# Borda/pyImSegm

Hardware: AMD Instinct MI355X
Metric: Mpixels/s end-to-end SLIC+fts+GC, 2048x2048 RGB; % HBM roofline (higher is better)
Workload: dtype f64; 1 GPU; single 2048x2048 RGB uint8 per GPU, SLIC(sp_size=46, K=2025, 10 sweeps) + colour mean/std/energy + 3-class alpha-expansion GC (gc_regul=2.0, edge=model), pre-fitted GMM, host numpy in -> segm int32 in host numpy (BASELINE configs[1]); bench_config=2, images_per_launch_chain=1, images_in_flight_per_gpu=4, hardware_queues=4, input_memory=pageable numpy, input_ring=default (one rank: measured in round 4), parallelism=images sharded over 1 GPU(s), 4 in flight per GPU (one HIP stream each)

## Files before the change

### pyimsegm_amd/build.py

```python
import os
import subprocess
import sys

HERE = os.path.dirname(os.path.abspath(__file__))
CSRC = os.path.join(HERE, 'csrc')
LIB = os.path.join(HERE, 'libimsegm_hip.so')
SOURCES = ['api.hip', 'api_image2d.hip', 'api_texture.hip', 'api_volume.hip', 'api_fused.hip', 'api_natives.hip', 'batch.hip', 'slic_pre.hip', 'slic.hip', 'connectivity.hip', 'stats.hip', 'graph.hip', 'graphcut.hip', 'texture.hip', 'volume.hip', 'terms.hip', 'natives.hip', 'median.hip', 'output.hip']
HEADERS = ['common.h', 'slic.h', 'session.h', os.path.join('..', '..', 'include', 'imsegm_hip.h')]
FLAGS = ['--offload-arch=gfx950', '-O3', '-std=c++17', '-fPIC', '-ffp-contract=off', '-fvisibility=hidden',
         '-Wall', '-Wno-unused-function', '-Wno-pass-failed']


def _stale(target, deps):
    if not os.path.exists(target):
        return True
    t = os.path.getmtime(target)
    return any(os.path.getmtime(d) > t for d in deps)


def build(force=False, verbose=True):
    hipcc = os.environ.get('HIPCC', '/opt/rocm/bin/hipcc')
    objdir = os.path.join(HERE, 'build')
    os.makedirs(objdir, exist_ok=True)
    headers = [os.path.join(CSRC, h) for h in HEADERS]
    objs = []
    procs = []
    for src in SOURCES:
        spath = os.path.join(CSRC, src)
        obj = os.path.join(objdir, src.replace('.hip', '.o'))
        objs.append(obj)
        if force or _stale(obj, [spath] + headers):
            cmd = [hipcc] + FLAGS + ['-c', spath, '-o', obj]
            if verbose:
                print(' '.join(cmd), flush=True)
            procs.append((src, subprocess.Popen(cmd)))
    for src, p in procs:
        if p.wait() != 0:
            raise RuntimeError('hipcc failed on %s' % src)
    if force or procs or _stale(LIB, objs):
        cmd = [hipcc, '--offload-arch=gfx950', '-shared', '-fPIC', '-o', LIB] + objs
        if verbose:
            print(' '.join(cmd), flush=True)
        subprocess.check_call(cmd)
    return LIB


if __name__ == '__main__':
    build(force='--force' in sys.argv)
```

### pyimsegm_amd/csrc/api.hip

```cpp
#include "../../include/imsegm_hip.h"
#include "slic.h"

#include <atomic>
#include <cstdio>
#include <cstdlib>
#include <cstring>
#include <vector>

namespace imsegm {

static thread_local std::string g_error;

void set_error(const std::string &msg) { g_error = msg; }

bool hip_ok(hipError_t e, const char *what, const char *file, int line)
{
    if (e == hipSuccess) return true;
    char buf[512];
    snprintf(buf, sizeof(buf), "HIP error %d (%s) in `%s` at %s:%d", (int)e, hipGetErrorString(e), what, file, line);
    g_error = buf;
    return false;
}

static Knobs read_knobs()
{
    auto flag = [](const char *n) { return getenv(n) != nullptr; };
    auto num = [](const char *n, int dflt) { const char *e = getenv(n); return e ? atoi(e) : dflt; };
    Knobs k;
    k.slic_graph = flag("IMSEGM_SLIC_GRAPH");
    k.pre_3pass = flag("IMSEGM_PRE_3PASS");
    k.separate_finalize = flag("IMSEGM_SEPARATE_FINALIZE");
    k.fuse_finalize = flag("IMSEGM_FUSE_FINALIZE");
    k.conn_general = flag("IMSEGM_CONN_GENERAL");
    k.gc_no_topo_regs = flag("IMSEGM_GC_NO_TOPO_REGS");
    k.sep_wide_tile = flag("IMSEGM_SEP_WIDE_TILE");
    k.cc_merge_full = flag("IMSEGM_CC_MERGE_FULL");
    k.label_general = flag("IMSEGM_LABEL_GENERAL");
    k.terms_one_workgroup = flag("IMSEGM_TERMS_ONE_WORKGROUP");
    k.adjacency_table = flag("IMSEGM_ADJACENCY_TABLE");
    k.brick_cap = num("IMSEGM_BRICK_CAP", 0);
    k.gc_lds_level = num("IMSEGM_GC_LDS_LEVEL", 4);
    k.gc_threads = num("IMSEGM_GC_THREADS", 0);
    k.gc_grid_min_sites = num("IMSEGM_GC_GRID_MIN_SITES", 0);
    k.gc_grid_blocks = num("IMSEGM_GC_GRID_BLOCKS", 0);
    k.gc_one_workgroup = flag("IMSEGM_GC_ONE_WORKGROUP");
    k.gc_grid_test_absent = flag("IMSEGM_GC_GRID_TEST_ABSENT");
    k.fused_bitmap_mb = num("IMSEGM_FUSED_BITMAP_MB", 0);
    const char *d = getenv("IMSEGM_PHASE_DUMP");
    k.phase_dump = d ? d : "";
    return k;
}
static std::atomic<const Knobs *> g_knobs{ nullptr };
const Knobs &knobs()
{
    const Knobs *k = g_knobs.load(std::memory_order_acquire);
    if (!k) {
        const Knobs *fresh = new Knobs(read_knobs());
        if (g_knobs.compare_exchange_strong(k, fresh, std::memory_order_acq_rel)) k = fresh;
        else delete fresh;
    }
    return *k;
}
void reload_knobs() { g_knobs.store(new Knobs(read_knobs()), std::memory_order_release); }

}

#include "session.h"

std::atomic<bool> g_runtime_started{ false };

extern "C" {

int imsegm_host_alloc(size_t bytes, void **ptr_out)
{
    g_runtime_started.store(true);
    if (!ptr_out) {
        set_error("null argument");
        return -1;
    }
    HIP_TRY(hipHostMalloc(ptr_out, bytes ? bytes : 1, hipHostMallocDefault));
    return 0;
}

void imsegm_host_free(void *ptr)
{
    if (ptr) (void)hipHostFree(ptr);
}

int imsegm_device_alloc(int device, size_t bytes, void **ptr_out)
{
    g_runtime_started.store(true);
    if (!ptr_out) {
        set_error("null argument");
        return -1;
    }
    HIP_TRY(hipSetDevice(device));
    HIP_TRY(hipMalloc(ptr_out, bytes ? bytes : 1));
    return 0;
}

void imsegm_device_free(void *ptr)
{
    if (ptr) (void)hipFree(ptr);
}

int imsegm_set_device(int device)
{
    g_runtime_started.store(true);
    HIP_TRY(hipSetDevice(device));
    return 0;
}

int imsegm_ctx_stream(imsegm_ctx *ctx, void **stream_out)
{
    if (bind(ctx)) return -1;
    *stream_out = ctx->stream;
    return 0;
}

int imsegm_ctx_copy(imsegm_ctx *ctx, void *dst, const void *src, size_t bytes, int synchronize)
{
    if (bind(ctx)) return -1;
    HIP_TRY(hipMemcpyAsync(dst, src, bytes, hipMemcpyDefault, ctx->stream));
    if (synchronize) HIP_TRY(hipStreamSynchronize(ctx->stream));
    return 0;
}

const char *imsegm_last_error(void) { return g_error.c_str(); }
int imsegm_version(void) { return 100; }

// ... 59 lines not shown
    ctx->device = device;
    HIP_TRY(hipStreamCreateWithFlags(&ctx->stream, hipStreamNonBlocking));
    *ctx_out = ctx;
    return 0;
}

void imsegm_ctx_destroy(imsegm_ctx *ctx)
{
    if (!ctx) return;
    (void)hipSetDevice(ctx->device);
    ctx->collect();
    for (auto e : ctx->pool) (void)hipEventDestroy(e);
    ctx->gc_buf.release();
    ctx->aux_buf.release();
    if (ctx->pinned_ev) (void)hipEventDestroy(ctx->pinned_ev);
    if (ctx->pinned) (void)hipHostFree(ctx->pinned);
    if (ctx->stream) (void)hipStreamDestroy(ctx->stream);
    delete ctx;
}

int imsegm_ctx_synchronize(imsegm_ctx *ctx)
{
    if (bind(ctx)) return -1;
    HIP_TRY(hipStreamSynchronize(ctx->stream));
    return 0;
}

int imsegm_ctx_profile_enable(imsegm_ctx *ctx, int enable)
{
    if (bind(ctx)) return -1;
    ctx->collect();
    ctx->profile = enable != 0;
    return 0;
}

int imsegm_ctx_profile_reset(imsegm_ctx *ctx)
{
    if (bind(ctx)) return -1;
    ctx->collect();
    for (int i = 0; i < PG_COUNT; ++i) {
        ctx->acc_ms[i] = 0;
        ctx->acc_n[i] = 0;
    }
    return 0;
}

int imsegm_ctx_profile_get(imsegm_ctx *ctx, int group, double *total_ms_out, int *count_out)
{
    if (bind(ctx)) return -1;
    if (group < 0 || group >= PG_COUNT) {
        set_error("bad profile group");
        return -1;
    }
    ctx->collect();
    *total_ms_out = ctx->acc_ms[group];
    *count_out = ctx->acc_n[group];
    return 0;
}

int imsegm_image2d_create(imsegm_ctx *ctx, int height, int width, imsegm_image2d **img_out)
{
    if (bind(ctx)) return -1;
    if (height <= 0 || width <= 0 || (long)height * width > 0x3fffffffL) {
        set_error("bad image size");
        return -1;
    }
    imsegm_image2d *im = new imsegm_image2d();
    im->ctx = ctx;
    im->H = height;
    im->W = width;
    im->n = (size_t)height * width;
    *img_out = im;
    return 0;
}

void imsegm_image2d_destroy(imsegm_image2d *im)
{
    if (!im) return;
    (void)hipSetDevice(im->ctx->device);
    (void)hipStreamSynchronize(im->ctx->stream);
    DevBuf *all[] = { &im->img, &im->labA, &im->labB, &im->nearest, &im->labels, &im->conn_i32, &im->conn_u8, &im->small,
                      &im->cent, &im->tiles, &im->feat, &im->graph, &im->gather_lut, &im->gather_out_i, &im->gather_out_f,
                      &im->tex_planes, &im->tex_resp, &im->tex_small, &im->vol_cent, &im->annot, &im->hist, &im->featK, &im->seg,
                      &im->gseg, &im->narrow };
    for (auto b : all) b->release();
    if (im->slic_fail_host) (void)hipHostFree(im->slic_fail_host);
    if (im->slic_exec) (void)hipGraphExecDestroy(im->slic_exec);
    delete im;
}

int imsegm_image2d_upload(imsegm_image2d *im, const void *host_pixels, int dtype)
{
    if (!im || bind(im->ctx)) return -1;
    if (wrong_kind(im, false)) return -1;
    im->tex_ready = false;
    size_t es = dtype == IMSEGM_U8 ? 1 : dtype == IMSEGM_F32 ? 4 : dtype == IMSEGM_F64 ? 8 : 0;
    if (!es) {
        set_error("unsupported dtype");
        return -1;
    }
    size_t bytes = im->n * 3 * es;
    if (im->img.ensure(bytes + 16)) return -1;
    HIP_TRY(hipMemcpyAsync(im->img.p, host_pixels, bytes, hipMemcpyHostToDevice, im->ctx->stream));
    if (!is_pinned(host_pixels)) HIP_TRY(hipStreamSynchronize(im->ctx->stream));
    im->dtype = dtype;
    im->feat_mask = 0;
    im->place_F = 0;
    return 0;
}

long imsegm_debug_conn_general_runs(void) { return conn_general_runs(); }

void imsegm_debug_reload_env(void) { reload_knobs(); }

long imsegm_debug_gc_grid_fallbacks(void) { return gc_grid_fallbacks(); }

int imsegm_debug_slic_sweep_runs(long *persistent_runs_out, long *fallback_runs_out)
{
    slic_sweep_counters(persistent_runs_out, fallback_runs_out);
    return 0;
}

int imsegm_image2d_all_finite(imsegm_image2d *im, int *all_finite_out)
{
    if (!im || !all_finite_out || bind(im->ctx)) return -1;
    if (im->dtype < 0 || !im->img.p) {
        set_error("all_finite needs an uploaded image or volume");
        return -1;
    }
    *all_finite_out = 1;
    if (im->dtype == IMSEGM_U8) return 0;
    hipStream_t st = im->ctx->stream;
    if (ensure_small(im)) return -1;
    unsigned int *count = reinterpret_cast<unsigned int *>(im->small.as<unsigned char>() + 256);
    const size_t values = im->is_volume ? im->n : im->n * 3;
    if (launch_count_nonfinite(im->img.p, im->dtype, values, count, st)) return -1;
    unsigned int bad = 0;
    HIP_TRY(hipMemcpyAsync(&bad, count, sizeof(bad), hipMemcpyDeviceToHost, st));
    HIP_TRY(hipStreamSynchronize(st));
    *all_finite_out = bad == 0;
    return 0;
}

int imsegm_image2d_device_ptr(imsegm_image2d *im, int which, void **ptr_out)
{
    if (!im || !ptr_out) {
        set_error("null argument");
        return -1;
    }
    DevBuf *b = which == 0 ? &im->labels : which == 1 ? &im->gather_out_i : which == 2 ? &im->gather_out_f : nullptr;
    if (!b || !b->p) {
        set_error("device_ptr: buffer not available");
        return -1;
    }
    *ptr_out = b->p;
    return 0;
}


}
```

### pyimsegm_amd/csrc/api_fused.hip

```cpp
#include "session.h"

extern "C" {

int imsegm_cut_general_graph(imsegm_ctx *ctx, const int32_t *edges, int n_edges, const double *edge_weights,
                             const double *unary_cost, int n_sites, int n_labels, const double *pairwise_cost,
                             int n_iter, int32_t *labels_out, int64_t *energy_out)
{
    if (bind(ctx)) return -1;
    const int K = n_sites, C = n_labels, E = n_edges;
    if (K < 1 || C < 1 || E < 0) {
        set_error("cut_general_graph: bad sizes");
        return -1;
    }
    for (int j = 0; j < E; ++j) {
        int a = edges[2 * j], b = edges[2 * j + 1];
        if (a < 0 || b >= K || a >= b) {
            set_error("cut_general_graph: edges must satisfy 0 <= edges[:,0] < edges[:,1] < n_sites");
            return -1;
        }
    }
    for (int a = 0; a < C; ++a)
        for (int b = 0; b < C; ++b)
            if (pairwise_cost[a * C + b] != pairwise_cost[b * C + a]) {
                set_error("Cost matrix not square or not symmetric");
// ... 409 lines not shown
        return -1;
    }
    memset(host, 0, up_bytes);
    reinterpret_cast<int32_t *>(host + o_misc)[0] = K;
    memcpy(host + o_pw, pairwise, (size_t)C * C * 8);
    int32_t *si = reinterpret_cast<int32_t *>(host + o_sm);
    int smax = 0;
    double pmax = -DBL_MAX;
    for (int i = 0; i < C * C; ++i) {
        si[i] = (int32_t)(pairwise[i] * 100);
        smax = std::max(smax, std::abs(si[i]));
        pmax = std::max(pmax, pairwise[i]);
    }
    const int metric = smooth_is_metric(si, C);
    if (classes_lut) memcpy(host + o_cl, classes_lut, (size_t)C * 4);
    if (gmm) {
        if (gmm->scaler_mean) memcpy(host + o_sc, gmm->scaler_mean, (size_t)F * 8);
        if (gmm->scaler_scale) memcpy(host + o_sc + (size_t)F * 8, gmm->scaler_scale, (size_t)F * 8);
        memcpy(host + o_pc, gmm->prec_chol, (size_t)C * FF * 8);
        memcpy(host + o_mp, gmm->mu_proj, (size_t)C * F * 8);
        memcpy(host + o_ld, gmm->log_det, (size_t)C * 8);
        memcpy(host + o_lw, gmm->log_weights, (size_t)C * 8);
    } else {
        memcpy(host + o_pr, proba, (size_t)K * C * 8);
    }
    HIP_TRY(hipMemcpyAsync(dev + d_par, host, up_bytes, hipMemcpyHostToDevice, st));
    ctx->mark_stage_in_flight();
    int32_t *misc = reinterpret_cast<int32_t *>(dev + d_misc);
    int32_t *K_dev = misc, *E_dev = misc + 1, *status = misc + 2;
    long long *energy = reinterpret_cast<long long *>(dev + d_misc + 16);
    double *scalars = reinterpret_cast<double *>(dev + d_misc + 64);
    if (prepared) E_dev = nullptr;
    else if (graph_enqueue(im, g, K_dev, E_dev)) return -1;
    unsigned char *gb = im->gseg.as<unsigned char>();
    int32_t *ghead = reinterpret_cast<int32_t *>(gb + g.o_head);
    if (!E_dev) E_dev = ghead + 1;
    int32_t *edges = reinterpret_cast<int32_t *>(gb + g.o_edges);
    double *centres = reinterpret_cast<double *>(gb + g.o_cent);
    int32_t *arc_start = reinterpret_cast<int32_t *>(gb + g.o_as), *arc_to = reinterpret_cast<int32_t *>(gb + g.o_at);
    int32_t *arc_rev = reinterpret_cast<int32_t *>(gb + g.o_ar), *edge_arc = reinterpret_cast<int32_t *>(gb + g.o_ea);
    TermsArgs a;
    memset(&a, 0, sizeof(a));
    a.Kp = K_dev; a.K_cap = K; a.Ep = E_dev; a.edge_capacity = Ecap; a.F = F; a.C = C;
    a.features = need_features ? im->featK.as<double>() : nullptr;
    a.gmm = gmm ? 1 : 0;
    if (gmm) {
        a.scaler_mean = gmm->scaler_mean ? reinterpret_cast<double *>(dev + d_par + o_sc) : nullptr;
        a.scaler_scale = gmm->scaler_scale ? reinterpret_cast<double *>(dev + d_par + o_sc) + F : nullptr;
        a.prec_chol = reinterpret_cast<double *>(dev + d_par + o_pc);
        a.mu_proj = reinterpret_cast<double *>(dev + d_par + o_mp);
        a.log_det = reinterpret_cast<double *>(dev + d_par + o_ld);
        a.log_w = reinterpret_cast<double *>(dev + d_par + o_lw);
        a.const_term = gmm->const_term;
    }
    a.proba = reinterpret_cast<double *>(dev + d_proba);
    a.edge_type = edge_code; a.spatial_norm = spatial_norm; a.edge_cost = edge_cost;
    a.edges = edges; a.centres = centres; a.ndim = ndim;
    a.edge_dist = reinterpret_cast<double *>(dev + d_edist); a.edge_len = reinterpret_cast<double *>(dev + d_elen);
    a.unary = reinterpret_cast<double *>(dev + d_unary); a.weights = reinterpret_cast<double *>(dev + d_w);
    a.pairwise = reinterpret_cast<double *>(dev + d_par + o_pw); a.pairwise_max = pmax;
    a.unary_i = reinterpret_cast<int32_t *>(dev + d_unary_i); a.weights_i = reinterpret_cast<int32_t *>(dev + d_wi);
    a.smooth_max = smax; a.status = status; a.scalars = scalars; a.fstd = reinterpret_cast<double *>(dev + d_fstd);
    int spt = ctx->begin(PG_TERMS);
    if (launch_gc_terms(a, st)) return -1;
    ctx->end(spt);
    int32_t *glab = reinterpret_cast<int32_t *>(dev + d_gl);
    int spg = ctx->begin(PG_GC);
    if (use_graphcut) {
        GcProblem p;
        p.K = K; p.C = C; p.E = Ecap; p.E_dev = E_dev;
        p.edges = edges; p.w = a.weights_i; p.unary = a.unary_i; p.smooth = reinterpret_cast<int32_t *>(dev + d_par + o_sm);
        p.metric = metric;
        if (launch_alpha_expansion(p, arc_start, arc_to, arc_rev, edge_arc, -1, glab, energy, status + 1, dev + d_work, st))
            return -1;
    } else if (launch_unary_argmin(a.unary, K_dev, K, C, glab, st)) {
        return -1;
    }
    ctx->end(spg);
    int32_t *lut = reinterpret_cast<int32_t *>(dev + d_lut);
    if (launch_label_lut(glab, K_dev, K, classes_lut ? reinterpret_cast<int32_t *>(dev + d_par + o_cl) : nullptr, lut, st)) return -1;
    if (im->gather_out_i.ensure(n * 4)) return -1;
    const bool want_soft = soft_out != nullptr || (debug_out && debug_out->keep_soft_on_device);
    if (want_soft && im->gather_out_f.ensure(n * C * 8)) return -1;
    int spq = ctx->begin(PG_GATHER);
    if (launch_gather_labels(lut, im->labels.as<int32_t>(), n, im->gather_out_i.as<int32_t>(), st)) return -1;
    if (want_soft && launch_gather_proba(a.proba, C, im->labels.as<int32_t>(), n, im->gather_out_f.as<double>(), st)) return -1;
    ctx->end(spq);
    const bool segm_u8 = debug_out && debug_out->segm_u8, soft_f32 = debug_out && debug_out->soft_f32;
    if ((segm_u8 && segm_out) || (soft_f32 && soft_out)) {
        const size_t off_soft = (n + 255) & ~(size_t)255;
        if (im->narrow.ensure(off_soft + n * C * 4 + 64)) return -1;
        unsigned char *nb = im->narrow.as<unsigned char>();
        if (segm_u8 && segm_out) {
            if (launch_narrow_labels_u8(im->gather_out_i.as<int32_t>(), nb, n, st)) return -1;
            HIP_TRY(hipMemcpyAsync(segm_out, nb, n, hipMemcpyDeviceToHost, st));
            segm_out = nullptr;
        }
        if (soft_f32 && soft_out) {
            float *f32 = reinterpret_cast<float *>(nb + off_soft);
            if (launch_narrow_soft_f32(im->gather_out_f.as<double>(), f32, n * C, st)) return -1;
            HIP_TRY(hipMemcpyAsync(soft_out, f32, n * C * 4, hipMemcpyDeviceToHost, st));
            soft_out = nullptr;
        }
    }
    if (segm_out) HIP_TRY(hipMemcpyAsync(segm_out, im->gather_out_i.p, n * 4, hipMemcpyDeviceToHost, st));
    if (soft_out) HIP_TRY(hipMemcpyAsync(soft_out, im->gather_out_f.p, n * C * 8, hipMemcpyDeviceToHost, st));
    if (graph_labels_out) HIP_TRY(hipMemcpyAsync(graph_labels_out, glab, (size_t)K * 4, hipMemcpyDeviceToHost, st));
    if (proba_out) HIP_TRY(hipMemcpyAsync(proba_out, a.proba, (size_t)K * C * 8, hipMemcpyDeviceToHost, st));
    int32_t hmisc[4] = { 0, 0, 0, 0 }, hgraph[4] = { 0, 0, 0, 0 };
    HIP_TRY(hipMemcpyAsync(hmisc, misc, sizeof(hmisc), hipMemcpyDeviceToHost, st));
    if (prepared || g.table) HIP_TRY(hipMemcpyAsync(hgraph, ghead, sizeof(hgraph), hipMemcpyDeviceToHost, st));
    if (debug_out) {
        if (debug_out->unary) HIP_TRY(hipMemcpyAsync(debug_out->unary, a.unary, (size_t)K * C * 8, hipMemcpyDeviceToHost, st));
        if (debug_out->unary_int) HIP_TRY(hipMemcpyAsync(debug_out->unary_int, a.unary_i, (size_t)K * C * 4, hipMemcpyDeviceToHost, st));
        if (debug_out->centres) HIP_TRY(hipMemcpyAsync(debug_out->centres, centres, (size_t)K * ndim * 8, hipMemcpyDeviceToHost, st));
        if (debug_out->energy) HIP_TRY(hipMemcpyAsync(debug_out->energy, energy, 8, hipMemcpyDeviceToHost, st));
    }
    HIP_TRY(hipStreamSynchronize(st));
    const int E = prepared ? hgraph[1] : hmisc[1];
    if (g.table && hgraph[2]) {
        set_error("segment: too many labels for the fused path (a label with more than 64 neighbours in the neighbour table)");
        return IMSEGM_E_FUSED_PATH;
    }
    if (debug_out) {
        debug_out->n_edges = E;
        const int Ec = std::min(E, debug_out->edge_capacity);
        if (Ec > 0) {
            if (debug_out->edges) HIP_TRY(hipMemcpy(debug_out->edges, edges, (size_t)Ec * 8, hipMemcpyDeviceToHost));
            if (debug_out->edge_weights) HIP_TRY(hipMemcpy(debug_out->edge_weights, a.weights, (size_t)Ec * 8, hipMemcpyDeviceToHost));
            if (debug_out->edge_weights_int) HIP_TRY(hipMemcpy(debug_out->edge_weights_int, a.weights_i, (size_t)Ec * 4, hipMemcpyDeviceToHost));
        }
    }
    if (edges_found) *edges_found = E;
    if (hmisc[2] & 2) {
        set_error("segment: more graph edges than the edge table holds");
        return -2;
    }
    if (use_graphcut && (hmisc[2] & 1)) {
        set_error("cut_general_graph: smoothness term is larger than GCO_MAX_ENERGYTERM");
        return -1;
    }
    if (use_graphcut && hmisc[3] != 0) {
        set_error("alpha_expansion: max-flow did not converge");
        return -1;
    }
    return 0;
}


int imsegm_image2d_run_color(imsegm_image2d *im, const void *host_pixels, int dtype, int minmax_normalize, int n_segments,
                             double compactness, const double *taps, int radius, int max_iter, int start_label, int slic_zero,
                             int feature_mask, const imsegm_gmm *gmm, int n_classes, const double *pairwise, int edge_type,
                             double edge_cost, int use_graphcut, const int32_t *classes_lut, int32_t *segm_out, double *soft_out,
                             int *n_labels_out)
{
    if (imsegm_image2d_upload(im, host_pixels, dtype)) return -1;
    int n_labels = 0;
    if (imsegm_image2d_slic(im, minmax_normalize, n_segments, compactness, taps, radius, taps, radius, taps, radius, max_iter, 1, 0.5,
                            3.0, start_label, 0, slic_zero, &n_labels))
        return -1;
    if (n_labels_out) *n_labels_out = n_labels;
    if (imsegm_image2d_features_color(im, feature_mask, nullptr)) return -1;
    return imsegm_image2d_segment(im, gmm, nullptr, n_classes, pairwise, edge_type, edge_cost, use_graphcut, classes_lut, segm_out,
                                  soft_out, nullptr, nullptr, nullptr);
}



}
```

### pyimsegm_amd/csrc/common.h

```cpp
#pragma once
#include <hip/hip_runtime.h>
#include <stdint.h>
#include <string>
#include <type_traits>

#define IMSEGM_WAVE 64

namespace imsegm {

void set_error(const std::string &msg);
bool hip_ok(hipError_t e, const char *what, const char *file, int line);

#define HIP_TRY(expr)                                                                   \
    do {                                                                                \
        if (!::imsegm::hip_ok((expr), #expr, __FILE__, __LINE__)) return -1;            \
    } while (0)

struct Knobs {
    bool slic_graph, pre_3pass, separate_finalize, fuse_finalize, conn_general, gc_no_topo_regs,
        adjacency_table,
        cc_merge_full,
        terms_one_workgroup,
        label_general,
        sep_wide_tile;
    int brick_cap;
    int gc_lds_level;
    int gc_threads;
    int gc_grid_min_sites;
    int gc_grid_blocks;
    bool gc_one_workgroup;
    bool gc_grid_test_absent;
    int fused_bitmap_mb;
    std::string phase_dump;
};
const Knobs &knobs();
void reload_knobs();

constexpr int IMSEGM_MAX_DEVICES = 64;
__host__ __device__ static inline int cdiv(long a, long b) { return (int)((a + b - 1) / b); }

struct ZBatch {
    int nz = 1;
    size_t zs = 0;
};
template <typename T> __device__ __forceinline__ T *zshift(T *p, size_t zs)
{
    typedef typename std::conditional<std::is_const<T>::value, const char, char>::type byte_t;
    T *const shifted = reinterpret_cast<T *>(reinterpret_cast<byte_t *>(p) + (size_t)blockIdx.z * zs);
    return p ? shifted : nullptr;
}
template <typename T> __device__ __forceinline__ T *zshift_nn(T *p, size_t zs)
{
    typedef typename std::conditional<std::is_const<T>::value, const char, char>::type byte_t;
    return reinterpret_cast<T *>(reinterpret_cast<byte_t *>(p) + (size_t)blockIdx.z * zs);
}
#define ZSHIFT(p, zs) (p) = ::imsegm::zshift((p), (zs))
#define ZSHIFT_NN(p, zs) (p) = ::imsegm::zshift_nn((p), (zs))

__device__ __forceinline__ double det_cbrt(double x)
{
    long long i = __double_as_longlong(x);
    i = 0x553ef0ff289dd796LL - i / 3;
    double y = __longlong_as_double(i);
    const double third = 1.0 / 3.0;
#pragma unroll
    for (int it = 0; it < 5; ++it) {
        double y3 = y * y * y;
        double r = 1.0 - x * y3;
        y = y + y * (r * third);
    }
    double yy = y * y;
    double c = x * yy;
    double e = c * c * c - x;
    c = c - e * (yy * third);
    return c;
}

__device__ __forceinline__ double div_by_const_in_range(double x, double c, double rc)
{
    const double q = x * rc;
    const double r = fma(-q, c, x);
    return fma(r, rc, q);
}
#define DIV_CONST_IN_RANGE(x, C) ::imsegm::div_by_const_in_range((x), (C), 1.0 / (C))

__device__ __forceinline__ double det_pow24(double t)
{
    long long i = __double_as_longlong(t);
    i = 0x4cb8a8c154c985f0LL - i / 5;
    double y = __longlong_as_double(i);
#pragma unroll
    for (int it = 0; it < 5; ++it) {
        double y2 = y * y;
        double y5 = y2 * y2 * y;
        double r = 1.0 - t * y5;
        y = y + y * (r * 0.2);
    }
    double p = t * y;
    return p * p * p;
}

__device__ __forceinline__ void rgb2lab_px(double r, double g, double b, double &L, double &A, double &B)
{
    double lin[3] = { r, g, b };
#pragma unroll
    for (int c = 0; c < 3; ++c) {
        double v = lin[c];
        lin[c] = (v > 0.04045) ? det_pow24((v + 0.055) / 1.055) : v / 12.92;
    }
    double X = lin[0] * 0.412453 + lin[1] * 0.357580 + lin[2] * 0.180423;
    double Y = lin[0] * 0.212671 + lin[1] * 0.715160 + lin[2] * 0.072169;
    double Z = lin[0] * 0.019334 + lin[1] * 0.119193 + lin[2] * 0.950227;
    double f[3] = { X / 0.95047, Y / 1.0, Z / 1.08883 };
#pragma unroll
    for (int c = 0; c < 3; ++c) {
// ... 360 lines not shown
```

### pyimsegm_amd/csrc/output.hip

```cpp
#include "slic.h"

namespace imsegm {

struct Rects {
    int r0[4], r1[4], c0[4], c1[4];
};

__global__ void __launch_bounds__(256) k_rect_minmax(const int32_t *__restrict__ labels, int W, Rects rc, int32_t *__restrict__ out)
{
    const int q = blockIdx.y;
    const int h = rc.r1[q] - rc.r0[q], w = rc.c1[q] - rc.c0[q];
    const long area = (long)max(h, 0) * max(w, 0);
    int mn = 0x7fffffff, mx = (int)0x80000000;
    for (long i = (long)blockIdx.x * 256 + threadIdx.x; i < area; i += (long)gridDim.x * 256) {
        const int y = rc.r0[q] + (int)(i / w), x = rc.c0[q] + (int)(i % w);
        const int v = labels[(size_t)y * W + x];
        mn = min(mn, v);
        mx = max(mx, v);
    }
#pragma unroll
    for (int off = 32; off > 0; off >>= 1) {
        mn = min(mn, __shfl_xor(mn, off, 64));
        mx = max(mx, __shfl_xor(mx, off, 64));
    }
// ... 18 lines not shown
    for (long i = (long)blockIdx.x * 256 + threadIdx.x; i < area; i += (long)gridDim.x * 256) {
        const int y = rc.r0[q] + (int)(i / w), x = rc.c0[q] + (int)(i % w);
        const int v = labels[(size_t)y * W + x];
        if (v < 0 || v >= nb) continue;
        if (lds) atomicAdd(&lh[v], 1u);
        else atomicAdd(&hist[v], 1ull);
    }
    if (lds) {
        __syncthreads();
        for (int i = threadIdx.x; i < nb; i += 256)
            if (lh[i]) atomicAdd(&hist[i], (unsigned long long)lh[i]);
    }
}

__global__ void __launch_bounds__(256) k_swap_labels(int32_t *__restrict__ labels, size_t n, int a, int b)
{
    for (size_t i = (size_t)blockIdx.x * 256 + threadIdx.x; i < n; i += (size_t)gridDim.x * 256) {
        const int v = labels[i];
        labels[i] = v == a ? b : (v == b ? a : v);
    }
}

int launch_boundary_minmax(const int32_t *labels, int W, const int rects[16], int32_t *out2_dev, hipStream_t st)
{
    Rects rc;
    for (int q = 0; q < 4; ++q) { rc.r0[q] = rects[4 * q]; rc.r1[q] = rects[4 * q + 1]; rc.c0[q] = rects[4 * q + 2]; rc.c1[q] = rects[4 * q + 3]; }
    const int32_t init[2] = { 0x7fffffff, (int32_t)0x80000000 };
    HIP_TRY(hipMemcpyAsync(out2_dev, init, sizeof(init), hipMemcpyHostToDevice, st));
    hipLaunchKernelGGL(k_rect_minmax, dim3(64, 4), 256, 0, st, labels, W, rc, out2_dev);
    HIP_TRY(hipGetLastError());
    return 0;
}

int launch_boundary_hist(const int32_t *labels, int W, const int rects[16], unsigned long long *hist_dev, int nb, hipStream_t st)
{
    Rects rc;
    for (int q = 0; q < 4; ++q) { rc.r0[q] = rects[4 * q]; rc.r1[q] = rects[4 * q + 1]; rc.c0[q] = rects[4 * q + 2]; rc.c1[q] = rects[4 * q + 3]; }
    HIP_TRY(hipMemsetAsync(hist_dev, 0, (size_t)nb * sizeof(unsigned long long), st));
    hipLaunchKernelGGL(k_rect_hist, dim3(64, 4), 256, 0, st, labels, W, rc, hist_dev, nb);
    HIP_TRY(hipGetLastError());
    return 0;
}

int launch_swap_labels(int32_t *labels, size_t n, int a, int b, hipStream_t st)
{
    hipLaunchKernelGGL(k_swap_labels, (int)std::min<size_t>(cdiv((long)n, 256 * 8), 4096), 256, 0, st, labels, n, a, b);
    HIP_TRY(hipGetLastError());
    return 0;
}

__global__ void __launch_bounds__(256) k_narrow_i32_u8(const int32_t *__restrict__ src, uint8_t *__restrict__ dst, size_t n)
{
    const size_t n4 = n / 4;
    for (size_t i = (size_t)blockIdx.x * 256 + threadIdx.x; i < n4; i += (size_t)gridDim.x * 256) {
        const int4 v = reinterpret_cast<const int4 *>(src)[i];
        reinterpret_cast<uint32_t *>(dst)[i] = (uint32_t)(uint8_t)v.x | ((uint32_t)(uint8_t)v.y << 8) | ((uint32_t)(uint8_t)v.z << 16) | ((uint32_t)(uint8_t)v.w << 24);
    }
    if (blockIdx.x == 0)
        for (size_t i = n4 * 4 + threadIdx.x; i < n; i += 256) dst[i] = (uint8_t)src[i];
}
__global__ void __launch_bounds__(256) k_narrow_f64_f32(const double *__restrict__ src, float *__restrict__ dst, size_t n)
{
    const size_t n2 = n / 2;
    for (size_t i = (size_t)blockIdx.x * 256 + threadIdx.x; i < n2; i += (size_t)gridDim.x * 256) {
        const double2 v = reinterpret_cast<const double2 *>(src)[i];
        reinterpret_cast<float2 *>(dst)[i] = make_float2((float)v.x, (float)v.y);
    }
    if (blockIdx.x == 0 && threadIdx.x == 0 && (n & 1)) dst[n - 1] = (float)src[n - 1];
}

int launch_narrow_labels_u8(const int32_t *src, uint8_t *dst, size_t n, hipStream_t st)
{
    hipLaunchKernelGGL(k_narrow_i32_u8, (int)std::min<size_t>(std::max<size_t>(cdiv((long)n, 1024), 1), 4096), 256, 0, st, src, dst, n);
    HIP_TRY(hipGetLastError());
    return 0;
}
int launch_narrow_soft_f32(const double *src, float *dst, size_t n, hipStream_t st)
{
    hipLaunchKernelGGL(k_narrow_f64_f32, (int)std::min<size_t>(std::max<size_t>(cdiv((long)n, 512), 1), 8192), 256, 0, st, src, dst, n);
    HIP_TRY(hipGetLastError());
    return 0;
}

template <typename T>
__global__ void __launch_bounds__(256) k_count_nonfinite(const T *__restrict__ src, size_t n, unsigned int *count)
{
    unsigned int bad = 0;
    for (size_t i = (size_t)blockIdx.x * 256 + threadIdx.x; i < n; i += (size_t)gridDim.x * 256) bad += !isfinite((double)src[i]);
    if (__syncthreads_or(bad) && bad) atomicAdd(count, bad);
}

int launch_count_nonfinite(const void *src, int dtype, size_t n, unsigned int *count_dev, hipStream_t st)
{
    HIP_TRY(hipMemsetAsync(count_dev, 0, sizeof(unsigned int), st));
    const int grid = (int)std::min<size_t>(std::max<size_t>(cdiv((long)n, 2048), 1), 8192);
    if (dtype == DT_F32) hipLaunchKernelGGL(k_count_nonfinite<float>, grid, 256, 0, st, (const float *)src, n, count_dev);
    else if (dtype == DT_F64) hipLaunchKernelGGL(k_count_nonfinite<double>, grid, 256, 0, st, (const double *)src, n, count_dev);
    HIP_TRY(hipGetLastError());
    return 0;
}

}
```

### pyimsegm_amd/csrc/session.h

```cpp
#pragma once
#include "../../include/imsegm_hip.h"
#include "slic.h"

#include <atomic>
#include <cstdio>
#include <cstdlib>
#include <cstring>
#include <vector>

namespace imsegm {

struct DevBuf {
    void *p = nullptr;
    size_t cap = 0;
    int ensure(size_t bytes)
    {
        if (bytes <= cap) return 0;
        if (p) HIP_TRY(hipFree(p));
        p = nullptr;
        cap = 0;
        size_t want = bytes + bytes / 8 + 256;
        HIP_TRY(hipMalloc(&p, want));
        cap = want;
        return 0;
// ... 47 lines not shown
        if (bytes > pinned_cap) {
            if (pinned) (void)hipHostFree(pinned);
            pinned = nullptr;
            pinned_cap = 0;
            size_t want = bytes + bytes / 2 + 4096;
            if (hipHostMalloc(&pinned, want, hipHostMallocDefault) != hipSuccess) return nullptr;
            pinned_cap = want;
        }
        return pinned;
    }

    hipEvent_t get_event()
    {
        if (!pool.empty()) {
            hipEvent_t e = pool.back();
            pool.pop_back();
            return e;
        }
        hipEvent_t e;
        (void)hipEventCreate(&e);
        return e;
    }
    int begin(int group)
    {
        if (!profile) return -1;
        Span s;
        s.group = group;
        s.a = get_event();
        s.b = get_event();
        (void)hipEventRecord(s.a, stream);
        spans.push_back(s);
        return (int)spans.size() - 1;
    }
    void end(int id)
    {
        if (id >= 0) (void)hipEventRecord(spans[id].b, stream);
    }
    void pair(int group, hipEvent_t *a, hipEvent_t *b)
    {
        Span s;
        s.group = group;
        s.a = get_event();
        s.b = get_event();
        spans.push_back(s);
        *a = s.a;
        *b = s.b;
    }
    void collect()
    {
        if (spans.empty()) return;
        (void)hipStreamSynchronize(stream);
        for (auto &s : spans) {
            float ms = 0;
            if (hipEventElapsedTime(&ms, s.a, s.b) == hipSuccess) {
                acc_ms[s.group] += ms;
                acc_n[s.group] += 1;
            }
            pool.push_back(s.a);
            pool.push_back(s.b);
        }
        spans.clear();
    }
};

struct GraphPlan {
    int K = 0, Ecap = 0, cap = 0, words = 0;
    bool table = false;
    size_t o_head = 0, o_edges = 0, o_as = 0, o_at = 0, o_ar = 0, o_ea = 0, o_deg = 0, o_dlow = 0, o_es = 0, o_cent = 0, o_present = 0,
           o_store = 0, o_cacc = 0, o_wp = 0, bytes = 0;
};

struct imsegm_image2d {
    imsegm_ctx *ctx = nullptr;
    int D = 1, H = 0, W = 0;
    size_t n = 0;
    int dtype = -1;
    int n_labels = 0;
    bool have_labels = false;
    bool labels_connected = false;
    bool tex_ready = false;
    bool is_volume = false;
    double vol_off = 0.0, vol_scale = 1.0;
    DevBuf img, labA, labB, nearest, labels, conn_i32, conn_u8, small, cent, tiles, feat, graph, gather_lut, gather_out_i, gather_out_f,
        tex_planes, tex_resp, tex_small, vol_cent, annot, hist, featK, seg, gseg, narrow;
    GraphPlan gplan;
    bool graph_ready = false;
    int *slic_fail_host = nullptr;
    int feat_mask = 0, feat_F = 0;
    int place_F = 0, place_col = 0;
    hipGraphExec_t slic_exec = nullptr;
    std::vector<unsigned char> slic_key;
};

inline int wrong_kind(const imsegm_image2d *im, bool want_volume)
{
    if (im && im->is_volume != want_volume) {
        set_error(want_volume ? "this call needs a volume session" : "this call needs a 2-D colour image session");
        return 1;
    }
    return 0;
}

extern std::atomic<bool> g_runtime_started;

inline int bind(imsegm_ctx *ctx)
{
    if (!ctx) {
        set_error("null context");
        return -1;
    }
    HIP_TRY(hipSetDevice(ctx->device));
    return 0;
}

inline int ensure_small(imsegm_image2d *im)
{
    if (im->small.cap >= 4096) return 0;
    if (im->small.ensure(4096)) return -1;
    HIP_TRY(hipMemsetAsync(im->small.p, 0, 4096, im->ctx->stream));
    return 0;
}

struct GridAxis {
    long start, step;
    bool all;
};
inline void regular_grid3(const long shape[3], long n_points, GridAxis out[3])
{
    int order[3] = { 0, 1, 2 };
    std::stable_sort(order, order + 3, [&](int a, int b) { return shape[a] < shape[b]; });
    double sorted_dims[3] = { (double)shape[order[0]], (double)shape[order[1]], (double)shape[order[2]] };
    double space = sorted_dims[0] * sorted_dims[1] * sorted_dims[2];
    if (space <= (double)n_points) {
        for (int i = 0; i < 3; ++i) out[i] = { 0, 1, true };
        return;
    }
    double steps[3];
    for (int i = 0; i < 3; ++i) steps[i] = pow(space / (double)n_points, 1.0 / 3);
    bool any_small = false;
    for (int i = 0; i < 3; ++i) any_small |= sorted_dims[i] < steps[i];
    if (any_small) {
        for (int dim = 0; dim < 3; ++dim) {
            steps[dim] = sorted_dims[dim];
            double sp = 1.0;
            for (int j = dim + 1; j < 3; ++j) sp *= sorted_dims[j];
            if (dim < 2) {
                double s = pow(sp / (double)n_points, 1.0 / (3 - dim - 1));
                for (int j = dim + 1; j < 3; ++j) steps[j] = s;
            }
            bool ok = true;
            for (int j = 0; j < 3; ++j) ok &= sorted_dims[j] >= steps[j];
            if (ok) break;
        }
    }
    for (int i = 0; i < 3; ++i) {
        long start = (long)floor(steps[i] / 2.0);
        long step = (long)nearbyint(steps[i]);
        out[order[i]] = { start, step, false };
    }
}

inline int fill_taps(Taps &t, const double *w, int r)
{
    t.r = -1;
    for (int i = 0; i < 17; ++i) t.w[i] = 0;
    if (r < 0 || !w) return 0;
    if (r > 16) {
// ... 64 lines not shown
```

### pyimsegm_amd/csrc/slic.h

```cpp
#pragma once
#include "common.h"
#include <algorithm>
#include <cfloat>
#include <cmath>

namespace imsegm {

enum { DT_U8 = 0, DT_F64 = 1, DT_F32 = 2 };

struct Taps {
    int r;
    double w[17];
};

constexpr int SLIC_TILE_X = 64, SLIC_TILE_Y = 32, SLIC_MAXC = 64;
struct Cand {
    double cy, cx, cL, ca, cb;
    int4 win;
    int k;
    float ry, rx;
    float fL, fa, fb;
    double mdc;
};

// ... 94 lines not shown
                              int32_t *n_edges_dev, hipStream_t st);
int launch_edge_extract(const uint32_t *bitmap, int K, int words, int32_t *rowcount, int32_t *edges_out, int edge_capacity,
                        int32_t *n_edges_dev, hipStream_t st);

struct ConnWork {
    int32_t *parent;
    int32_t *csize;
    int32_t *newlabel;
    int32_t *adjptr;
    int32_t *queue;
    uint8_t *visited;
    int32_t *blocksum;
    int32_t *list;
    int32_t *counters;
    int32_t *slotmap;
    int32_t *bbox;
    int32_t *dense;
    size_t dense_ints;
};
constexpr size_t CONN_DENSE_INTS = 2 * 65536 + 16 * 4096;
constexpr int CONN_TILE_PIXELS = 64 * 32, CONN_TILE_SLOTS = 256;
static inline size_t conn_i32_bytes(size_t n, size_t H = 0, size_t W = 0)
{
    const size_t n_tiles = ((W + 63) / 64) * ((H + 31) / 32);
    return n * 4 * 8 + ((n / 4096) + 64) * 4 + 256 + (CONN_DENSE_INTS + n_tiles * (3 * CONN_TILE_SLOTS + 1)) * 4;
}
int launch_label_connected(int32_t *labels_inout, size_t n, int n_labels, int32_t *first, uint32_t *bitmap, int32_t *blocksum,
                           int32_t *counters, int32_t *total_dev, hipStream_t st);
long conn_general_runs();
long gc_grid_fallbacks();
int launch_enforce_connectivity(const int32_t *labels_in, int D, int H, int W, long min_size, long max_size,
                                int start_label, ConnWork w, int32_t *labels_out, int *n_labels_out_host,
                                hipStream_t st);
int launch_enforce_connectivity_batch(const int32_t *labels_in, int H, int W, long min_size, long max_size, int start_label, ConnWork w,
                                      int32_t *labels_out, int *n_labels_out, hipStream_t st, ZBatch zb, int32_t *stage_dev);

int launch_label_hist(const int32_t *labels, const int32_t *annot, size_t n, int K, int nb, unsigned long long *hist,
                      hipStream_t st);
int launch_color_stats(const void *img, int dtype, const int32_t *labels, int H, int W, int K, double maxabs,
                       int want_var, long long *acc, double *mean_out, double *energy_out, double *var_out,
                       float *mean32_scratch, hipStream_t st, int planar = 0, int prescale = 0, double mul = 1.0,
                       double div = 1.0, long plane_stride = -1, const double *ssq_dev = nullptr, ZBatch zb = ZBatch(),
                       const double *minmax_dev = nullptr);

struct SepJob {
    double *resp;
    const double *taps;
    int groups, rank, merge;
};
constexpr int SEP_MAX_JOBS = 5;
struct SepJobs {
    int n;
    SepJob job[SEP_MAX_JOBS];
};
int launch_battery_dense(const double *planes, int H, int W, const double *wgt_dev, int nk, int radius, double clip, double *resp,
                         hipStream_t st, int P, int parity);
size_t sep_sumsq_scratch(int H, int W, int P, int radius, int jobs);
int launch_battery_sep(const double *planes, int H, int W, int radius, double clip, const SepJobs &jobs, hipStream_t st, int P,
                       double *ssq_scratch, double *const *ssq_out);
int launch_response_sumsq(const double *resp, size_t count, double *partial, double *sumsq_dev, hipStream_t st);
int launch_texture_prepare(const void *img, int dtype, int H, int W, const double *taps_dev, int radius,
                           const double *mix_dev, double *planes, double *tmpA, double *tmpB, hipStream_t st, double *fullpad);
int launch_texture_prepare_volume(const void *vol, int dtype, int P, int H, int W, const double *taps_dev, int radius, double *planes,
                                  double *tmpA, double *tmpB, hipStream_t st, double *fullpad);
int launch_filter_battery(const double *planes, int H, int W, const double *wgt_dev, int nk, int radius, double clip,
                          double *resp, double *partial, double *sumsq_dev, hipStream_t st, int P = 3, const double *sep_dev = nullptr,
                          int sep_groups = 0, int sep_rank = 0, int parity = 0);

int launch_adjacency_centres(const int32_t *labels, int H, int W, int K, uint32_t *bitmap, long long *cacc,
                             int32_t *edges_out, int edge_capacity, int32_t *n_edges_dev, double *centres_out,
                             uint8_t *present_out, int32_t *rowcount, hipStream_t st);
int launch_adjacency_bitmap(const int32_t *labels, int H, int W, int K, uint32_t *bitmap, long long *cacc, double *centres_out,
                            uint8_t *present_out, hipStream_t st, ZBatch zb = ZBatch());
int launch_gather_labels(const int32_t *lut, const int32_t *idx, size_t n, int32_t *out, hipStream_t st, ZBatch zb = ZBatch());
int launch_zero(void *ptr, size_t bytes, hipStream_t st, ZBatch zb);
int launch_copy_rows(void *dst, size_t dst_stride, const void *src, size_t src_stride, size_t bytes, int rows, hipStream_t st);
int launch_gather_proba(const double *lut, int C, const int32_t *idx, size_t n, double *out, hipStream_t st);

int launch_boundary_minmax(const int32_t *labels, int W, const int rects[16], int32_t *out2_dev, hipStream_t st);
int launch_boundary_hist(const int32_t *labels, int W, const int rects[16], unsigned long long *hist_dev, int nb, hipStream_t st);
int launch_swap_labels(int32_t *labels, size_t n, int a, int b, hipStream_t st);
int launch_narrow_labels_u8(const int32_t *src, uint8_t *dst, size_t n, hipStream_t st);
int launch_narrow_soft_f32(const double *src, float *dst, size_t n, hipStream_t st);
int launch_count_nonfinite(const void *src, int dtype, size_t n, unsigned int *count_dev, hipStream_t st);

int launch_gradient_image(const void *src, void *dst, int dtype, int S, int H, int W, int C, hipStream_t st);
size_t median_scratch_bytes(size_t n, int K);
int launch_segment_median(const void *img, int dtype, int C, size_t n, const int32_t *labels, int K, void *scratch, size_t scratch_bytes,
                          double *out, hipStream_t st);

int launch_label_hist2d(const int16_t *segm, int H, int W, const int32_t *windows, int P, const int16_t *selem, int SH, int SW,
                        int nb_labels, unsigned int *hist, hipStream_t st);
int launch_ray_features_binary2d(const int8_t *seg, int H, int W, const int32_t *positions, int P, const float *grad, int A, int edge,
                                 float *out, hipStream_t st);

struct GcProblem {
    int K, C, E;
    const int32_t *E_dev = nullptr;
    const int32_t *K_dev = nullptr;
    const int32_t *edges;
    const int32_t *w;
    const int32_t *unary;
    const int32_t *smooth;
    int metric = 0;
};
static inline int smooth_is_metric(const int32_t *s, int C)
{
    for (int a = 0; a < C; ++a) {
        if (s[a * C + a] != 0) return 0;
        for (int b = 0; b < C; ++b)
            if (s[a * C + b] < 0 || s[a * C + b] != s[b * C + a]) return 0;
    }
    for (int a = 0; a < C; ++a)
        for (int b = 0; b < C; ++b)
            for (int c = 0; c < C; ++c)
                if ((long long)s[a * C + b] > (long long)s[a * C + c] + (long long)s[c * C + b]) return 0;
    return 1;
}
int launch_alpha_expansion(GcProblem p, const int32_t *arc_start, const int32_t *arc_to, const int32_t *arc_rev,
                           const int32_t *edge_arc, int n_iter, int32_t *labels_dev, long long *energy_dev,
                           int32_t *status_dev, void *work, hipStream_t st, ZBatch zb = ZBatch());
size_t alpha_expansion_work_bytes(int K, int E);

struct TermsArgs {
    const int *Kp;
    int K_cap;
    const int *Ep;
    int edge_capacity;
    int F, C;
    const double *features;
    int gmm;
    const double *scaler_mean, *scaler_scale;
    const double *prec_chol;
    const double *mu_proj;
    const double *log_det;
    const double *log_w;
    double const_term;
    double *proba;
    int edge_type;
    int spatial_norm;
    double edge_cost;
    const int32_t *edges;
    const double *centres;
    int ndim;
    double *edge_dist, *edge_len;
    double *unary;
    double *weights;
    const double *pairwise;
    double pairwise_max;
    int32_t *unary_i, *weights_i;
    int smooth_max;
    int32_t *status;
    double *scalars;
    double *fstd;
    size_t zs;
};
int launch_features_assemble(const double *mean, const double *energy, const double *var, int K, int mask, double *out,
                             hipStream_t st, int row_stride = 0, int col0 = 0, ZBatch zb = ZBatch());
int launch_graph_csr(uint32_t *bitmap, const int *K_dev, int K_cap, int words, int32_t *wordprefix, int32_t *deg, int32_t *deg_low,
                     int32_t *arc_start, int32_t *edge_start, int32_t *n_edges_dev, int edge_capacity, int32_t *edges,
                     int32_t *arc_to, int32_t *arc_rev, int32_t *edge_arc, hipStream_t st, ZBatch zb = ZBatch());
int launch_graph_csr_table(int32_t *table, const int *K_dev, int K_cap, int cap, const int *overflow, int32_t *deg, int32_t *deg_low,
                           int32_t *arc_start, int32_t *edge_start, int32_t *n_edges_dev, int edge_capacity, int32_t *edges,
                           int32_t *arc_to, int32_t *arc_rev, int32_t *edge_arc, hipStream_t st);
int launch_gc_terms(const TermsArgs &a, hipStream_t st, int nz = 1);
int launch_unary_argmin(const double *unary, const int *K_dev, int K_cap, int C, int32_t *labels, hipStream_t st, ZBatch zb = ZBatch());
// ... 5 lines not shown
```

Before: 5575 Mpixels/s.

## Pack class map to 2-bit on device and widen on host threads

```diff
diff --git a/pyimsegm_amd/build.py b/pyimsegm_amd/build.py
--- a/pyimsegm_amd/build.py
+++ b/pyimsegm_amd/build.py
@@ -5,7 +5,7 @@
 HERE = os.path.dirname(os.path.abspath(__file__))
 CSRC = os.path.join(HERE, 'csrc')
 LIB = os.path.join(HERE, 'libimsegm_hip.so')
-SOURCES = ['api.hip', 'api_image2d.hip', 'api_texture.hip', 'api_volume.hip', 'api_fused.hip', 'api_natives.hip', 'batch.hip', 'slic_pre.hip', 'slic.hip', 'connectivity.hip', 'stats.hip', 'graph.hip', 'graphcut.hip', 'texture.hip', 'volume.hip', 'terms.hip', 'natives.hip', 'median.hip', 'output.hip']
+SOURCES = ['api.hip', 'api_image2d.hip', 'api_texture.hip', 'api_volume.hip', 'api_fused.hip', 'api_natives.hip', 'batch.hip', 'slic_pre.hip', 'slic.hip', 'connectivity.hip', 'stats.hip', 'graph.hip', 'graphcut.hip', 'texture.hip', 'volume.hip', 'terms.hip', 'natives.hip', 'median.hip', 'output.hip', 'widen.hip']
 HEADERS = ['common.h', 'slic.h', 'session.h', os.path.join('..', '..', 'include', 'imsegm_hip.h')]
 FLAGS = ['--offload-arch=gfx950', '-O3', '-std=c++17', '-fPIC', '-ffp-contract=off', '-fvisibility=hidden',
          '-Wall', '-Wno-unused-function', '-Wno-pass-failed']
diff --git a/pyimsegm_amd/csrc/api.hip b/pyimsegm_amd/csrc/api.hip
--- a/pyimsegm_amd/csrc/api.hip
+++ b/pyimsegm_amd/csrc/api.hip
@@ -46,6 +46,7 @@
     k.gc_one_workgroup = flag("IMSEGM_GC_ONE_WORKGROUP");
     k.gc_grid_test_absent = flag("IMSEGM_GC_GRID_TEST_ABSENT");
     k.fused_bitmap_mb = num("IMSEGM_FUSED_BITMAP_MB", 0);
+    k.segm_packed = num("IMSEGM_SEGM_PACKED", 1) != 0;
     const char *d = getenv("IMSEGM_PHASE_DUMP");
     k.phase_dump = d ? d : "";
     return k;
@@ -271,8 +272,9 @@
     DevBuf *all[] = { &im->img, &im->labA, &im->labB, &im->nearest, &im->labels, &im->conn_i32, &im->conn_u8, &im->small,
                       &im->cent, &im->tiles, &im->feat, &im->graph, &im->gather_lut, &im->gather_out_i, &im->gather_out_f,
                       &im->tex_planes, &im->tex_resp, &im->tex_small, &im->vol_cent, &im->annot, &im->hist, &im->featK, &im->seg,
-                      &im->gseg, &im->narrow };
+                      &im->gseg, &im->narrow, &im->packed };
     for (auto b : all) b->release();
+    if (im->packed_host) (void)hipHostFree(im->packed_host);
     if (im->slic_fail_host) (void)hipHostFree(im->slic_fail_host);
     if (im->slic_exec) (void)hipGraphExecDestroy(im->slic_exec);
     delete im;
diff --git a/pyimsegm_amd/csrc/api_fused.hip b/pyimsegm_amd/csrc/api_fused.hip
--- a/pyimsegm_amd/csrc/api_fused.hip
+++ b/pyimsegm_amd/csrc/api_fused.hip
@@ -515,11 +515,36 @@
     if (im->gather_out_i.ensure(n * 4)) return -1;
     const bool want_soft = soft_out != nullptr || (debug_out && debug_out->keep_soft_on_device);
     if (want_soft && im->gather_out_f.ensure(n * C * 8)) return -1;
+    const bool segm_u8 = debug_out && debug_out->segm_u8, soft_f32 = debug_out && debug_out->soft_f32;
+    const int pack_bits = (!segm_out || segm_u8 || !knobs().segm_packed) ? 0 : C <= 4 ? 2 : C <= 16 ? 4 : C <= 256 ? 8 : 0;
+    int32_t *widen_to = nullptr;
+    size_t pack_bytes = 0;
+    if (pack_bits) {
+        pack_bytes = packed_words(n, pack_bits) * 4;
+        if (im->packed.ensure(pack_bytes)) return -1;
+        if (pack_bytes > im->packed_host_cap) {
+            if (im->packed_host) HIP_TRY(hipHostFree(im->packed_host));
+            im->packed_host = nullptr;
+            im->packed_host_cap = 0;
+            HIP_TRY(hipHostMalloc((void **)&im->packed_host, pack_bytes, hipHostMallocDefault));
+            im->packed_host_cap = pack_bytes;
+        }
+    }
     int spq = ctx->begin(PG_GATHER);
-    if (launch_gather_labels(lut, im->labels.as<int32_t>(), n, im->gather_out_i.as<int32_t>(), st)) return -1;
+    if (pack_bits) {
+        if (launch_gather_labels_packed(lut, glab, im->labels.as<int32_t>(), n, pack_bits, im->gather_out_i.as<int32_t>(),
+                                        im->packed.as<uint32_t>(), st))
+            return -1;
+    } else if (launch_gather_labels(lut, im->labels.as<int32_t>(), n, im->gather_out_i.as<int32_t>(), st)) {
+        return -1;
+    }
     if (want_soft && launch_gather_proba(a.proba, C, im->labels.as<int32_t>(), n, im->gather_out_f.as<double>(), st)) return -1;
     ctx->end(spq);
-    const bool segm_u8 = debug_out && debug_out->segm_u8, soft_f32 = debug_out && debug_out->soft_f32;
+    if (pack_bits) {
+        HIP_TRY(hipMemcpyAsync(im->packed_host, im->packed.p, pack_bytes, hipMemcpyDeviceToHost, st));
+        widen_to = segm_out;
+        segm_out = nullptr;
+    }
     if ((segm_u8 && segm_out) || (soft_f32 && soft_out)) {
         const size_t off_soft = (n + 255) & ~(size_t)255;
         if (im->narrow.ensure(off_soft + n * C * 4 + 64)) return -1;
@@ -577,6 +602,11 @@
         set_error("alpha_expansion: max-flow did not converge");
         return -1;
     }
+    if (widen_to) {
+        int32_t values[256];
+        for (int c = 0; c < 256; ++c) values[c] = c < C ? (classes_lut ? classes_lut[c] : c) : 0;
+        widen_packed_labels(im->packed_host, n, pack_bits, values, widen_to);
+    }
     return 0;
 }
 
diff --git a/pyimsegm_amd/csrc/common.h b/pyimsegm_amd/csrc/common.h
--- a/pyimsegm_amd/csrc/common.h
+++ b/pyimsegm_amd/csrc/common.h
@@ -31,6 +31,7 @@
     bool gc_one_workgroup;
     bool gc_grid_test_absent;
     int fused_bitmap_mb;
+    bool segm_packed;
     std::string phase_dump;
 };
 const Knobs &knobs();
diff --git a/pyimsegm_amd/csrc/output.hip b/pyimsegm_amd/csrc/output.hip
--- a/pyimsegm_amd/csrc/output.hip
+++ b/pyimsegm_amd/csrc/output.hip
@@ -124,6 +124,45 @@
     return 0;
 }
 
+__global__ void __launch_bounds__(256)
+k_gather_i32_packed(const int32_t *__restrict__ lut, const int32_t *__restrict__ glab, const int32_t *__restrict__ idx, size_t n,
+                    int bits, int32_t *__restrict__ out, uint8_t *__restrict__ packed)
+{
+    const uint32_t mask = (1u << bits) - 1u;
+    const size_t t = (size_t)blockIdx.x * blockDim.x + threadIdx.x;
+    const size_t i = t * 4;
+    if (i >= n) return;
+    uint32_t v = 0;
+    if (i + 4 <= n) {
+        const int4 s = *reinterpret_cast<const int4 *>(idx + i);
+        *reinterpret_cast<int4 *>(out + i) = make_int4(lut[s.x], lut[s.y], lut[s.z], lut[s.w]);
+        v = ((uint32_t)glab[s.x] & mask) | (((uint32_t)glab[s.y] & mask) << bits) | (((uint32_t)glab[s.z] & mask) << (2 * bits)) |
+            (((uint32_t)glab[s.w] & mask) << (3 * bits));
+    } else {
+        for (int j = 0; i + j < n; ++j) {
+            const int32_t s = idx[i + j];
+            out[i + j] = lut[s];
+            v |= ((uint32_t)glab[s] & mask) << (bits * j);
+        }
+    }
+    if (bits == 2) packed[t] = (uint8_t)v;
+    else if (bits == 4) reinterpret_cast<uint16_t *>(packed)[t] = (uint16_t)v;
+    else reinterpret_cast<uint32_t *>(packed)[t] = v;
+}
+
+int launch_gather_labels_packed(const int32_t *lut, const int32_t *graph_labels, const int32_t *idx, size_t n, int bits, int32_t *out,
+                                uint32_t *packed, hipStream_t st)
+{
+    if (bits != 2 && bits != 4 && bits != 8) {
+        set_error("packed class map: 2, 4 or 8 bits per pixel");
+        return -1;
+    }
+    hipLaunchKernelGGL(k_gather_i32_packed, cdiv(cdiv((long)n, 4), 256), 256, 0, st, lut, graph_labels, idx, n, bits, out,
+                       reinterpret_cast<uint8_t *>(packed));
+    HIP_TRY(hipGetLastError());
+    return 0;
+}
+
 template <typename T>
 __global__ void __launch_bounds__(256) k_count_nonfinite(const T *__restrict__ src, size_t n, unsigned int *count)
 {
diff --git a/pyimsegm_amd/csrc/session.h b/pyimsegm_amd/csrc/session.h
--- a/pyimsegm_amd/csrc/session.h
+++ b/pyimsegm_amd/csrc/session.h
@@ -153,7 +153,9 @@
     bool is_volume = false;
     double vol_off = 0.0, vol_scale = 1.0;
     DevBuf img, labA, labB, nearest, labels, conn_i32, conn_u8, small, cent, tiles, feat, graph, gather_lut, gather_out_i, gather_out_f,
-        tex_planes, tex_resp, tex_small, vol_cent, annot, hist, featK, seg, gseg, narrow;
+        tex_planes, tex_resp, tex_small, vol_cent, annot, hist, featK, seg, gseg, narrow, packed;
+    unsigned char *packed_host = nullptr;
+    size_t packed_host_cap = 0;
     GraphPlan gplan;
     bool graph_ready = false;
     int *slic_fail_host = nullptr;
diff --git a/pyimsegm_amd/csrc/slic.h b/pyimsegm_amd/csrc/slic.h
--- a/pyimsegm_amd/csrc/slic.h
+++ b/pyimsegm_amd/csrc/slic.h
@@ -200,6 +200,10 @@
 int launch_swap_labels(int32_t *labels, size_t n, int a, int b, hipStream_t st);
 int launch_narrow_labels_u8(const int32_t *src, uint8_t *dst, size_t n, hipStream_t st);
 int launch_narrow_soft_f32(const double *src, float *dst, size_t n, hipStream_t st);
+inline size_t packed_words(size_t n, int bits) { return (n + 32 / bits - 1) / (32 / bits); }
+int launch_gather_labels_packed(const int32_t *lut, const int32_t *graph_labels, const int32_t *idx, size_t n, int bits, int32_t *out,
+                                uint32_t *packed, hipStream_t st);
+void widen_packed_labels(const uint8_t *src, size_t n, int bits, const int32_t *values, int32_t *dst);
 int launch_count_nonfinite(const void *src, int dtype, size_t n, unsigned int *count_dev, hipStream_t st);
 
 int launch_gradient_image(const void *src, void *dst, int dtype, int S, int H, int W, int C, hipStream_t st);
diff --git a/pyimsegm_amd/csrc/widen.hip b/pyimsegm_amd/csrc/widen.hip
--- /dev/null
+++ b/pyimsegm_amd/csrc/widen.hip
@@ -0,0 +1,172 @@
+#include "slic.h"
+
+#include <emmintrin.h>
+#include <pthread.h>
+#include <sched.h>
+
+#include <algorithm>
+#include <atomic>
+#include <condition_variable>
+#include <cstdint>
+#include <cstring>
+#include <deque>
+#include <mutex>
+#include <new>
+#include <thread>
+
+namespace imsegm {
+
+namespace {
+
+constexpr size_t WIDEN_PIECE = 1 << 16;
+constexpr size_t WIDEN_ALONE_BELOW = 1 << 18;
+
+struct WidenJob {
+    const uint8_t *src;
+    int32_t *dst;
+    size_t n;
+    int bits;
+    size_t pieces = 0, next = 0, done = 0;
+    alignas(16) int32_t tab[256 * 4];
+};
+
+void widen_piece(const WidenJob &j, size_t p0, size_t p1)
+{
+    const uint8_t *s = j.src;
+    int32_t *d = j.dst;
+    const int32_t *tab = j.tab;
+    const bool stream = (reinterpret_cast<uintptr_t>(d) & 15) == 0;
+    auto put = [&](size_t p, __m128i v) {
+        if (stream) _mm_stream_si128(reinterpret_cast<__m128i *>(d + p), v);
+        else _mm_storeu_si128(reinterpret_cast<__m128i *>(d + p), v);
+    };
+    size_t p = p0;
+    if (j.bits == 2) {
+        for (; p + 4 <= p1; p += 4) put(p, _mm_load_si128(reinterpret_cast<const __m128i *>(tab + 4 * s[p >> 2])));
+        for (; p < p1; ++p) d[p] = tab[4 * s[p >> 2] + (p & 3)];
+    } else if (j.bits == 4) {
+        for (; p + 4 <= p1; p += 4) {
+            const __m128i lo = _mm_loadl_epi64(reinterpret_cast<const __m128i *>(tab + 4 * s[p >> 1]));
+            const __m128i hi = _mm_loadl_epi64(reinterpret_cast<const __m128i *>(tab + 4 * s[(p >> 1) + 1]));
+            put(p, _mm_unpacklo_epi64(lo, hi));
+        }
+        for (; p < p1; ++p) d[p] = tab[4 * s[p >> 1] + (p & 1)];
+    } else {
+        for (; p + 4 <= p1; p += 4) put(p, _mm_setr_epi32(tab[4 * s[p]], tab[4 * s[p + 1]], tab[4 * s[p + 2]], tab[4 * s[p + 3]]));
+        for (; p < p1; ++p) d[p] = tab[4 * s[p]];
+    }
+    if (stream) _mm_sfence();
+}
+
+void widen_piece_index(const WidenJob &j, size_t c)
+{
+    widen_piece(j, c * WIDEN_PIECE, std::min(j.n, (c + 1) * WIDEN_PIECE));
+}
+
+int helper_count()
+{
+    cpu_set_t set;
+    CPU_ZERO(&set);
+    int cpus = sched_getaffinity(0, sizeof(set), &set) == 0 ? CPU_COUNT(&set) : 1;
+    return std::max(0, std::min(8, cpus - 1));
+}
+
+struct WidenPool {
+    std::mutex mu;
+    std::condition_variable work_cv, done_cv;
+    std::deque<WidenJob *> queue;
+    int helpers = 0;
+
+    void helper()
+    {
+        std::unique_lock<std::mutex> lk(mu);
+        for (;;) {
+            work_cv.wait(lk, [&] { return !queue.empty(); });
+            WidenJob *j = queue.front();
+            const size_t c = j->next++;
+            if (j->next == j->pieces) queue.pop_front();
+            lk.unlock();
+            widen_piece_index(*j, c);
+            lk.lock();
+            if (++j->done == j->pieces) done_cv.notify_all();
+        }
+    }
+
+    void run(WidenJob &j)
+    {
+        std::unique_lock<std::mutex> lk(mu);
+        queue.push_back(&j);
+        lk.unlock();
+        work_cv.notify_all();
+        lk.lock();
+        while (j.next < j.pieces) {
+            const size_t c = j.next++;
+            if (j.next == j.pieces) queue.erase(std::find(queue.begin(), queue.end(), &j));
+            lk.unlock();
+            widen_piece_index(j, c);
+            lk.lock();
+            ++j.done;
+        }
+        done_cv.wait(lk, [&] { return j.done == j.pieces; });
+    }
+};
+
+std::mutex g_pool_mu;
+WidenPool *g_pool = nullptr;
+
+void after_fork_in_child()
+{
+    new (&g_pool_mu) std::mutex();
+    g_pool = nullptr;
+}
+struct RegisterAtFork {
+    RegisterAtFork() { pthread_atfork(nullptr, nullptr, after_fork_in_child); }
+} g_register_at_fork;
+
+WidenPool *pool()
+{
+    WidenPool *p = __atomic_load_n(&g_pool, __ATOMIC_ACQUIRE);
+    if (p) return p;
+    std::lock_guard<std::mutex> lk(g_pool_mu);
+    p = __atomic_load_n(&g_pool, __ATOMIC_ACQUIRE);
+    if (p) return p;
+    p = new WidenPool();
+    const int want = helper_count();
+    for (int i = 0; i < want; ++i) {
+        try {
+            std::thread(&WidenPool::helper, p).detach();
+            ++p->helpers;
+        } catch (...) {
+            break;
+        }
+    }
+    __atomic_store_n(&g_pool, p, __ATOMIC_RELEASE);
+    return p;
+}
+
+}
+
+void widen_packed_labels(const uint8_t *src, size_t n, int bits, const int32_t *values, int32_t *dst)
+{
+    WidenJob j;
+    j.src = src;
+    j.dst = dst;
+    j.n = n;
+    j.bits = bits;
+    const int per = 8 / bits, mask = (1 << bits) - 1;
+    for (int b = 0; b < 256; ++b)
+        for (int k = 0; k < 4; ++k) j.tab[4 * b + k] = k < per ? values[(b >> (bits * k)) & mask] : 0;
+    j.pieces = (n + WIDEN_PIECE - 1) / WIDEN_PIECE;
+    if (n < WIDEN_ALONE_BELOW) {
+        widen_piece(j, 0, n);
+        return;
+    }
+    WidenPool *p = pool();
+    if (p->helpers == 0) {
+        widen_piece(j, 0, n);
+        return;
+    }
+    p->run(j);
+}
+
+}
```

After: 5890 Mpixels/s (median of 6 runs). 5.7% higher.
